# huangnengCSU/NanoSNP

Hardware: AMD Instinct MI355X
Metric: candidate SNP sites/sec (pileup encode + model fwd), 30x windows (higher is better)
Workload: dtype f32; 1 GPU; BASELINE configs[1]: pileup encode + PileupModel fwd, 1M synthetic 30x windows (G2) resident in HBM, batch=4096; batch=4096, windows_resident_per_gpu=1048576, streams=32, precision=fp32, parallelism=site-sharded x1, rooted gather of calls, world_size_observed=1, gather=torch

## Files before the change

nanosnp_amd/csrc/nsnp_api.hip:

```cpp
#include "nsnp_common.hpp"

#include <new>

extern "C" int nsnp_version(void) { return 101; }

extern "C" const char* nsnp_strerror(int code)
{
    switch (code) {
    case NSNP_OK: return "ok";
    case NSNP_EINVAL: return "invalid argument";
    case NSNP_ENOMEM: return "out of memory";
    case NSNP_EHIP: return "HIP runtime error";
    case NSNP_ENOWEIGHTS: return "weights not loaded";
    case NSNP_EARCH: return "device is not gfx950";
    case NSNP_ESHAPE: return "unsupported model dimensions";
    case NSNP_ENOTSUP: return "optional component unavailable (RCCL not found)";
    case NSNP_ECOMM: return "RCCL call failed";
    default: return "unknown error";
    }
}

static hipError_t g_create_err = hipSuccess;

extern "C" int nsnp_last_hip_error(const nsnp_ctx* ctx, const char** text)
{
    const hipError_t e = ctx ? ctx->last_err : g_create_err;
    if (text) *text = hipGetErrorString(e);
    return (int)e;
}

extern "C" int nsnp_ctx_create(int device, nsnp_ctx** out)
{
    if (!out) return NSNP_EINVAL;
    *out = nullptr;
    nsnp_ctx* ctx = new (std::nothrow) nsnp_ctx();
    if (!ctx) return NSNP_ENOMEM;
    memset((void*)ctx, 0, sizeof(*ctx));
    ctx->device = device;
    ctx->last_err = hipSuccess;
    ctx->chunk_sites = 32768;
    ctx->hap_chunk = 16384;
    ctx->precision = 0;
    ctx->hap_precision = 0;
    ctx->cat_precision = 0;
    ctx->cat_conv_lds = 1;
    ctx->cat_conv_pix2 = 1;
    ctx->hap_b3x = 1;
    ctx->tok_fused = 0;
    ctx->proj1_tiles = 4;
    ctx->fused_l1 = 1;
    ctx->l0_rs = 2;
    ctx->l0_weave = 1;
    ctx->l0_prestage = 1;
    ctx->l1_rs = 1;
    ctx->l1_stagger = 0;
    ctx->l1_weave = 1;
    ctx->head_rs = 1;
    ctx->rs_prio = 0;
    hipDeviceProp_t prop;
    hipError_t e = hipSetDevice(device);
    if (e == hipSuccess) e = hipGetDeviceProperties(&prop, device);
    if (e != hipSuccess) { g_create_err = e; delete ctx; return NSNP_EHIP; }
    if (strncmp(prop.gcnArchName, "gfx950", 6) != 0) { delete ctx; return NSNP_EARCH; }
    ctx->n_cu = prop.multiProcessorCount;
    *out = ctx;
    return NSNP_OK;
}

void nsnp_hap_free(nsnp_ctx* ctx);
int  nsnp_hap_reserve(nsnp_ctx* ctx);
void nsnp_cat_free(nsnp_ctx* ctx);
void nsnp_tok_free(nsnp_ctx* ctx);
void nsnp_train_free(nsnp_ctx* ctx);

constexpr size_t TIMER_MAX_PAIRS = 8192;

ScopedKernelTimer::ScopedKernelTimer(nsnp_ctx* c, int kernel, hipStream_t stream)
    : ctx(c), k(kernel), s(stream), stop_ev(nullptr), on(false)
{
    KernelTimer* t = c->timer;
    if (!t || !t->enabled || t->used[k] >= TIMER_MAX_PAIRS) return;
    if (t->used[k] == t->start[k].size()) {
        hipEvent_t a, b;
        if (hipEventCreate(&a) != hipSuccess) return;
        if (hipEventCreate(&b) != hipSuccess) { (void)hipEventDestroy(a); return; }
        t->start[k].push_back(a); t->stop[k].push_back(b);
    }
    const size_t i = t->used[k]++;
    (void)hipEventRecord(t->start[k][i], s);
    stop_ev = t->stop[k][i];
    on = true;
}
void ScopedKernelTimer::stop() { if (on) { (void)hipEventRecord(stop_ev, s); on = false; } }
ScopedKernelTimer::~ScopedKernelTimer() { stop(); }

extern "C" int nsnp_ctx_set_option(nsnp_ctx* ctx, const char* name, int64_t value)
{
    if (!ctx || !name) return NSNP_EINVAL;
    if (strcmp(name, "cat_precision") == 0) {
        if (value != 0 && value != 1 && value != 2) return NSNP_EINVAL;
        ctx->cat_precision = (int)value;
        return NSNP_OK;
    }
    if (strcmp(name, "tok_fused") == 0) {
        if (value != 0 && value != 1) return NSNP_EINVAL;
        ctx->tok_fused = (int)value;
        return NSNP_OK;
    }
    if (strcmp(name, "hap_b3x") == 0) {
        if (value != 0 && value != 1) return NSNP_EINVAL;
        ctx->hap_b3x = (int)value;
        return NSNP_OK;
    }
    if (strcmp(name, "cat_conv_pix2") == 0) {
        if (value != 0 && value != 1) return NSNP_EINVAL;
        ctx->cat_conv_pix2 = (int)value;
        return NSNP_OK;
    }
    if (strcmp(name, "cat_conv_lds") == 0) {
        if (value != 0 && value != 1) return NSNP_EINVAL;
        ctx->cat_conv_lds = (int)value;
        return NSNP_OK;
    }
    if (strcmp(name, "hap_precision") == 0) {
        if (value != 0 && value != 1 && value != 2) return NSNP_EINVAL;
        ctx->hap_precision = (int)value;
        return nsnp_hap_reserve(ctx);
    }
    if (strcmp(name, "hap_pass_sites") == 0) {
        if (value < 128 || value > 131072 || value % 128) return NSNP_EINVAL;
        const int64_t old = ctx->hap_chunk;
        ctx->hap_chunk = value;
        const int rc = nsnp_hap_reserve(ctx);
        if (rc) { ctx->hap_chunk = old; (void)nsnp_hap_reserve(ctx); }
        return rc;
    }
    if (strcmp(name, "pileup_precision") == 0) {
        if (value != 0 && value != 1 && value != 2) return NSNP_EINVAL;
        ctx->precision = (int)value;
        if (value == 2 && ctx->ws_h0 && ctx->ws_h0_floats < 192) return nsnp_ctx_reserve(ctx, ctx->chunk_sites);
        return NSNP_OK;
    }
    if (strcmp(name, "fused_l1") == 0) {
        if (value != 0 && value != 1) return NSNP_EINVAL;
        ctx->fused_l1 = (int)value;
        return NSNP_OK;
    }
    if (strcmp(name, "l0_register_stationary") == 0) {
        if (value != 0 && value != 1 && value != 2) return NSNP_EINVAL;
        ctx->l0_rs = (int)value;
        return NSNP_OK;
    }
    if (strcmp(name, "l1_register_stationary") == 0) {
        if (value != 0 && value != 1 && value != 2) return NSNP_EINVAL;
        ctx->l1_rs = (int)value;
        return NSNP_OK;
    }
    if (strcmp(name, "l0_input_weights_in_lds") == 0) {
        if (value != 0 && value != 1) return NSNP_EINVAL;
        ctx->l0_wx_lds = (int)value;
        return NSNP_OK;
    }
    if (strcmp(name, "static_priority") == 0) {
        if (value < 0 || value > 3) return NSNP_EINVAL;
        ctx->rs_prio = (int)value;
        return NSNP_OK;
    }
    if (strcmp(name, "head_split") == 0) {
        if (value != 0 && value != 1) return NSNP_EINVAL;
        ctx->head_rs = (int)value;
        return NSNP_OK;
    }
    if (strcmp(name, "l1_stagger") == 0) {
        if (value != 0 && value != 1) return NSNP_EINVAL;
        ctx->l1_stagger = (int)value;
        return NSNP_OK;
    }
    if (strcmp(name, "l1_weave") == 0) {
        if (value != 0 && value != 1) return NSNP_EINVAL;
        ctx->l1_weave = (int)value;
        return NSNP_OK;
    }
    if (strcmp(name, "l0_weave") == 0) {
        if (value != 0 && value != 1) return NSNP_EINVAL;
        ctx->l0_weave = (int)value;
        return NSNP_OK;
    }
    if (strcmp(name, "l0_prestage") == 0) {
        if (value != 0 && value != 1) return NSNP_EINVAL;
        ctx->l0_prestage = (int)value;
        return NSNP_OK;
    }
    if (strcmp(name, "l1_site_groups") == 0) {
        if (value != 0 && value != 1 && value != 2 && value != 4) return NSNP_EINVAL;
        ctx->l1_rs_groups = (int)value;
        return NSNP_OK;
    }
    if (strcmp(name, "l0_site_groups") == 0) {
        if (value != 0 && value != 1 && value != 2 && value != 4) return NSNP_EINVAL;
        ctx->l0_rs_groups = (int)value;
        return NSNP_OK;
    }
    if (strcmp(name, "fused_waves") == 0) {
        if (value != 0 && value != 4 && value != 8 && value != 12) return NSNP_EINVAL;
        ctx->fused_waves = (int)value;
        return NSNP_OK;
    }
    if (strcmp(name, "proj1_tiles") == 0) {
        if (value < 1 || value > 64) return NSNP_EINVAL;
        ctx->proj1_tiles = (int)value;
        return NSNP_OK;
    }
    if (strcmp(name, "recurrence_waves") == 0) {
        if (value != 0 && value != 1 && value != 2 && value != 4 && value != 8) return NSNP_EINVAL;
        ctx->force_wpb = (int)value;
        return NSNP_OK;
    }
    return NSNP_EINVAL;
}

extern "C" int nsnp_ctx_enable_timing(nsnp_ctx* ctx, int enable)
{
    if (!ctx) return NSNP_EINVAL;
    if (!ctx->timer) {
        ctx->timer = new (std::nothrow) KernelTimer();
        if (!ctx->timer) return NSNP_ENOMEM;
        for (int k = 0; k < NSNP_K_COUNT; ++k) ctx->timer->used[k] = 0;
    }
    ctx->timer->enabled = enable != 0;
    return NSNP_OK;
}

extern "C" int nsnp_ctx_read_timing(nsnp_ctx* ctx, int kernel, double* total_ms, int64_t* launches)
{
    if (!ctx || kernel < 0 || kernel >= NSNP_K_COUNT || !total_ms || !launches) return NSNP_EINVAL;
    *total_ms = 0.0; *launches = 0;
    KernelTimer* t = ctx->timer;
    if (!t) return NSNP_OK;
    for (size_t i = 0; i < t->used[kernel]; ++i) {
        NSNP_HIP(ctx, hipEventSynchronize(t->stop[kernel][i]));
        float ms = 0.f;
        NSNP_HIP(ctx, hipEventElapsedTime(&ms, t->start[kernel][i], t->stop[kernel][i]));
        *total_ms += ms; ++*launches;
    }
    t->used[kernel] = 0;
    return NSNP_OK;
}

static void free_ws(nsnp_ctx* ctx)
{
    if (ctx->ws_h0) (void)hipFree(ctx->ws_h0);
    if (ctx->ws_xp1) (void)hipFree(ctx->ws_xp1);
    if (ctx->ws_h1c) (void)hipFree(ctx->ws_h1c);
// ... 158 lines not shown
```

nanosnp_amd/csrc/nsnp_common.hpp:

```cpp
#pragma once

#include <hip/hip_runtime.h>
#include <stdint.h>
#include <stdlib.h>
#include <string.h>
#include <vector>

#include "nanosnp.h"

typedef float f32x4 __attribute__((ext_vector_type(4)));
typedef int   i32x4 __attribute__((ext_vector_type(4)));

#define NSNP_CDIV(a, b) (((a) + (b) - 1) / (b))

constexpr int PW = NSNP_PILEUP_WINDOW;
constexpr int PC = NSNP_PILEUP_CHANNELS;
constexpr int PH = 64;
constexpr int PG = 4 * PH;
constexpr int PCENTER = 16;
constexpr int PSTEPS1 = PCENTER + 1;


struct PileupWeightsDev {
    float* l0_whh[2];
    float* l0_wih[2];
    float* l0_wlast[2];
    void*  l0_wx[2];
    float* l1_wih[2];
    float* l1_bias[2];
    float* l1_bias_raw[2];
    float* l1_whh[2];
    float* proj_w;
    float* proj_b;
    float* dense_w;
    float* dense_b;
    float* head_w;
    float* head_b;
    float* arena;
    size_t arena_bytes;
    bool   loaded;
    float* head6_w;
    float* head6_b;
    bool   indel_loaded;
};

struct PileupWeightsF16 {
    void* l0_whh[2]; void* l0_wih_hi[2]; void* l0_wih_lo[2]; void* l1_wih[2]; void* l1_whh[2];
    void* l1f_hi[2]; void* l1f_lo[2]; float* l1f_bias;
    void* l0_wih_rs[2];
    void* l1_wih_rs[2]; void* l1_whh_rs[2];
    void* l0_whh_rs[2];
    void* proj_w; void* dense_w; void* head_w;
    void* arena; size_t arena_bytes; bool loaded;
};

struct PileupWeightsB3 {
    void* l0_whh[2]; void* l0_wih[2]; void* l1_wih[2]; void* l1_whh[2];
    void* proj_w; void* dense_w; void* head_w;
    float* proj_b; float* dense_b; float* head_b;
    void* arena; size_t arena_bytes; bool loaded;
};

struct HapWeightsDev;
struct CatWeightsDev;

enum { NSNP_K_L0 = 0, NSNP_K_PROJ1, NSNP_K_L1, NSNP_K_HEAD, NSNP_K_ENCODE, NSNP_K_HAPFEAT, NSNP_K_HAPLSTM, NSNP_K_CATCONV, NSNP_K_CAT,
       NSNP_K_HAPHEAD,
       NSNP_K_TRAIN_FWD, NSNP_K_TRAIN_BWD, NSNP_K_TRAIN_WGRAD,
       NSNP_K_COUNT };
struct KernelTimer {
    std::vector<hipEvent_t> start[NSNP_K_COUNT], stop[NSNP_K_COUNT];
    size_t used[NSNP_K_COUNT];
    bool enabled;
};

struct PostOut { uint8_t* gt_arg; uint8_t* zy_arg; float* gt_max; float* zy_max; };

struct nsnp_ctx {
    int device;
    int n_cu;
    hipError_t last_err;
    bool attr_set;
    bool attr_set_f16;
    bool attr_set_b3;
    int hap_b3x;
    int cat_conv_pix2;
    int cat_conv_lds;
    int cat_precision;
    int hap_precision;
    int precision;
    int fused_waves;
    int l0_rs;
    int l1_rs_groups;
    int l1_rs;
    int l0_rs_groups;
    int fused_l1;
    int proj1_tiles;
    int force_wpb;
    int l0_wx_lds;
    int rs_prio;
    int head_rs;
    int l1_stagger;
    int l0_weave;
    int l0_prestage;
    int l1_weave;
    int64_t chunk_sites;
    float*  ws_h0;
    int     ws_h0_floats;
    float*  ws_xp1;
    float*  ws_h1c;
    PileupWeightsDev pw;
    PileupWeightsF16 pw16;
    PileupWeightsB3 pwb3;
    HapWeightsDev* hw;
    void*  hap_ws; size_t hap_ws_bytes; int64_t hap_ws_chunk;
    int64_t hap_chunk;
    CatWeightsDev* cw;
    void*  cat_ws; size_t cat_ws_bytes;
    int64_t* sel_tmp; size_t sel_tmp_bytes;
    int64_t* fil_tmp; size_t fil_tmp_bytes;
    void* rec_tmp; size_t rec_tmp_bytes;
    void* evl_tmp; size_t evl_tmp_bytes;
    void* tr_ws; int64_t tr_sites;
    void* lab_tmp; size_t lab_tmp_bytes;
    void* tok_ws; size_t tok_ws_bytes;
    void* ctg_ws; size_t ctg_ws_bytes;
    int tok_fused;
    bool af_cached; uint64_t af_bits, af_t; int af_k, af_mode; uint32_t af_table_words[128];
    bool af2_cached; uint64_t af2_bits, af2_t; int af2_k, af2_mode; uint32_t af2_table_words[128];
    KernelTimer* timer;
    void* comm; int comm_rank, comm_world;
    bool comm_borrowed;
};

struct ScopedKernelTimer {
    nsnp_ctx* ctx; int k; hipStream_t s; hipEvent_t stop_ev; bool on;
    ScopedKernelTimer(nsnp_ctx* c, int kernel, hipStream_t stream);
    void stop();
    ~ScopedKernelTimer();
};

#define NSNP_HIP(ctx, call)                                                        \
    do {                                                                           \
        hipError_t e_ = (call);                                                    \
        if (e_ != hipSuccess) { (ctx)->last_err = e_; return NSNP_EHIP; }          \
    } while (0)

typedef float (*nsnp_wfun)(const void* user, int row, int k);
void nsnp_pack_image(float* img, int n_tiles, int n_j4, nsnp_wfun f, const void* user);

int nsnp_ctx_need_xp1(nsnp_ctx* ctx);

int nsnp_pileup_forward_impl(nsnp_ctx* ctx, const int32_t* x, const int64_t* center_idx,
                             int64_t N, float* gt, float* zy, const PostOut* post, bool* post_written, hipStream_t s);
int nsnp_pileup_pack_weights(nsnp_ctx* ctx, const float* const* w);
int nsnp_pileup_pack_indel_heads(nsnp_ctx* ctx, const float* const* w);
int nsnp_pileup_eval_impl(nsnp_ctx* ctx, const int32_t* x, const int64_t* center_idx, const uint8_t* cls, int64_t N, float* site_loss,
                          uint8_t* pred, int64_t* counters, float* logits, hipStream_t s);
void nsnp_pileup_eval_heads_launch(nsnp_ctx* ctx, int64_t n, const uint8_t* cls, float* site_loss, uint8_t* pred, int64_t* counters,
                                   float* logits, hipStream_t s);
int nsnp_hap_dims(const nsnp_ctx* ctx, int* n_gt, int* n_zy);
int nsnp_pileup_forward_f16x3(nsnp_ctx* ctx, const int32_t* x, const int64_t* center_idx,
                              int64_t N, float* gt, float* zy, hipStream_t s);
int nsnp_pileup_pack_weights_f16(nsnp_ctx* ctx, const float* const* w);
int nsnp_pileup_forward_bf16x3(nsnp_ctx* ctx, const int32_t* x, const int64_t* center_idx, int64_t N, float* gt, float* zy,
                               const PostOut* post, hipStream_t s);
int nsnp_pileup_pack_weights_bf16(nsnp_ctx* ctx, const float* const* w);
```

nanosnp_amd/csrc/pileup_forward.hip:

```cpp
#include "nsnp_common.hpp"
#include "nsnp_lstm_cell.hpp"
#include "nsnp_devclock.hpp"
#include "nsnp_bf16.hpp"
#include <type_traits>

namespace {

constexpr float LOG2E = 1.4426950408889634f;

__device__ __forceinline__ f32x4 mfma4(float a, float b, f32x4 c)
{
    return __builtin_amdgcn_mfma_f32_16x16x4f32(a, b, c, 0, 0, 0);
}
__device__ __forceinline__ float sigmoid_f(float x)
{
    return __builtin_amdgcn_rcpf(1.0f + __builtin_amdgcn_exp2f(-LOG2E * x));
}
__device__ __forceinline__ float tanh_f(float x)
{
    return __builtin_fmaf(-2.0f, __builtin_amdgcn_rcpf(1.0f + __builtin_amdgcn_exp2f((2.0f * LOG2E) * x)), 1.0f);
}

__device__ __forceinline__ float lstm_cell(float zi, float zf, float zg, float zo, float& c)
{
// ... 1526 lines not shown
        for (int u = 0; u < 2; ++u)
#pragma unroll
            for (int g = 0; g < 4; ++g) x2[4 * (2 * wave + u) + g][lane] = tanh_f(ad[u][g]);
        __syncthreads();
        f32x4 ah = bh;
        if (wave < 2) {
#pragma unroll
            for (int j = 0; j < 16; ++j)
#pragma unroll
                for (int e = 0; e < 4; ++e) ah = mfma4(Wh[j][e], x2[4 * j + e][lane], ah);
            if (wave == 1) x3[lane] = ah;
        }
        __syncthreads();
        if (wave == 0) {
            const f32x4 a1 = x3[lane];
            const float NEG = -3.0e38f;
            float g0[4], g1[4];
#pragma unroll
            for (int g = 0; g < 4; ++g) {
                g0[g] = ah[g];
                const bool is_gt = (q == 0) || (q == 1 && g == 0);
                g1[g] = is_gt ? a1[g] : NEG;
            }
            float mx = fmaxf(fmaxf(fmaxf(g0[0], g0[1]), fmaxf(g0[2], g0[3])), fmaxf(fmaxf(g1[0], g1[1]), fmaxf(g1[2], g1[3])));
            mx = fmaxf(mx, __shfl_xor(mx, 16));
            mx = fmaxf(mx, __shfl_xor(mx, 32));
            float e0[4], e1[4], sum = 0.f;
#pragma unroll
            for (int g = 0; g < 4; ++g) {
                e0[g] = __expf(g0[g] - mx);
                e1[g] = g1[g] > -1.0e38f ? __expf(g1[g] - mx) : 0.f;
                sum += e0[g] + e1[g];
            }
            sum += __shfl_xor(sum, 16);
            sum += __shfl_xor(sum, 32);
            const float z1 = a1[1], z2 = a1[2], z3 = a1[3];
            const float zm = fmaxf(z1, fmaxf(z2, z3));
            const float ez1 = __expf(z1 - zm), ez2 = __expf(z2 - zm), ez3 = __expf(z3 - zm);
            const float zs = ez1 + ez2 + ez3;
            float p0[4], p1[4];
#pragma unroll
            for (int g = 0; g < 4; ++g) { p0[g] = e0[g] / sum; p1[g] = e1[g] / sum; }
            const float pz1 = ez1 / zs, pz2 = ez2 / zs, pz3 = ez3 / zs;
            if (live) {
                float* gp = gt_prob + site * NSNP_GT_CLASSES;
#pragma unroll
                for (int g = 0; g < 4; ++g) gp[4 * q + g] = p0[g];
                if (q == 0) {
#pragma unroll
                    for (int g = 0; g < 4; ++g) gp[16 + g] = p1[g];
                }
                if (q == 1) {
                    gp[20] = p1[0];
                    float* zp = zy_prob + site * NSNP_ZY_CLASSES;
                    zp[0] = pz1; zp[1] = pz2; zp[2] = pz3;
                }
            }
            if (gt_arg) {
                float bv = p0[0]; int bi = 4 * q;
#pragma unroll
                for (int g = 1; g < 4; ++g) if (p0[g] > bv) { bv = p0[g]; bi = 4 * q + g; }
                if (q == 0) {
#pragma unroll
                    for (int g = 0; g < 4; ++g) if (p1[g] > bv) { bv = p1[g]; bi = 16 + g; }
                }
                if (q == 1 && p1[0] > bv) { bv = p1[0]; bi = 20; }
#pragma unroll
                for (int o = 16; o <= 32; o <<= 1) {
                    const float ov = __shfl_xor(bv, o); const int oi = __shfl_xor(bi, o);
                    if (ov > bv || (ov == bv && oi < bi)) { bv = ov; bi = oi; }
                }
                if (live && q == 0) { gt_arg[site] = (uint8_t)bi; gt_max[site] = bv; }
                if (live && q == 1) {
                    float zb = pz1; int zi = 0;
                    if (pz2 > zb) { zb = pz2; zi = 1; }
                    if (pz3 > zb) { zb = pz3; zi = 2; }
                    zy_arg[site] = (uint8_t)zi; zy_max[site] = zb;
                }
            }
        }
    }
}

__global__ void k_pileup_post(const float* __restrict__ gt, const float* __restrict__ zy,
                              const int32_t* __restrict__ x, int64_t N, uint8_t* gt_arg, uint8_t* zy_arg,
                              float* gt_max, float* zy_max, int32_t* depth)
{
    const int64_t n = (int64_t)blockIdx.x * blockDim.x + threadIdx.x;
    if (n >= N) return;
    const float* g = gt + n * NSNP_GT_CLASSES;
    int bi = 0; float bv = g[0];
    for (int i = 1; i < NSNP_GT_CLASSES; ++i) if (g[i] > bv) { bv = g[i]; bi = i; }
    gt_arg[n] = (uint8_t)bi; gt_max[n] = bv;
    const float* z = zy + n * NSNP_ZY_CLASSES;
    bi = 0; bv = z[0];
    for (int i = 1; i < NSNP_ZY_CLASSES; ++i) if (z[i] > bv) { bv = z[i]; bi = i; }
    zy_arg[n] = (uint8_t)bi; zy_max[n] = bv;
    if (depth) {
        const int32_t* c = x + n * (PW * PC) + PCENTER * PC;
        const int idx[8] = {0, 1, 2, 3, 9, 10, 11, 12};
        int d = 0;
        for (int k = 0; k < 8; ++k) { const int v = c[idx[k]]; if (v < 0) d -= v; }
        depth[n] = d;
    }
}

}

namespace {

inline int gate_row(int row)
{
    const int i = row >> 4, r = row & 15, qp = r >> 2, g = r & 3;
    return g * PH + 4 * i + qp;
}
struct MatRef { const float* w; int ld; const float* b0; const float* b1; };

float f_whh(const void* u, int row, int k) { const MatRef* m = (const MatRef*)u; return m->w[gate_row(row) * m->ld + k]; }
float f_wih0(const void* u, int row, int k) { const MatRef* m = (const MatRef*)u; return m->w[gate_row(row) * m->ld + k]; }
inline int h_store_col(int k) { const int j = k >> 2, q = k & 3; return (j >> 4) * 64 + 4 * (j & 15) + q; }
float f_wih1(const void* u, int row, int k) { const MatRef* m = (const MatRef*)u; return m->w[gate_row(row) * m->ld + h_store_col(k)]; }
float f_proj(const void* u, int row, int k) { const MatRef* m = (const MatRef*)u; return m->w[row * m->ld + h_store_col(k)]; }
inline int acc_col(int k) { const int j = k >> 2, q = k & 3; return 16 * (j >> 2) + 4 * q + (j & 3); }
float f_dense(const void* u, int row, int k) { const MatRef* m = (const MatRef*)u; return m->w[row * m->ld + acc_col(k)]; }
struct HeadRef { const float* gt; const float* zy; };
float f_head(const void* u, int row, int k)
{
    const HeadRef* m = (const HeadRef*)u;
    if (row < 21) return m->gt[row * 256 + acc_col(k)];
    if (row < 24) return m->zy[(row - 21) * 256 + acc_col(k)];
    return 0.f;
}

}

void nsnp_pack_image(float* img, int n_tiles, int n_j4, nsnp_wfun f, const void* user)
{
    for (int tile = 0; tile < n_tiles; ++tile)
        for (int j4 = 0; j4 < n_j4; ++j4)
            for (int lane = 0; lane < 64; ++lane)
                for (int e = 0; e < 4; ++e) {
                    const int row = 16 * tile + (lane & 15);
                    const int k = 4 * (4 * j4 + e) + (lane >> 4);
                    img[(((size_t)tile * n_j4 + j4) * 64 + lane) * 4 + e] = f(user, row, k);
                }
}

int nsnp_pileup_pack_weights(nsnp_ctx* ctx, const float* const* w)
{
    PileupWeightsDev& pw = ctx->pw;
    const size_t n_whh = 16 * 4 * 256, n_wih0 = 16 * 1 * 256, n_wlast = 16 * 64, n_wih1 = 16 * 8 * 256,
                 n_b1 = 16 * 256, n_proj = 8 * 8 * 256, n_pb = 8 * 256, n_dense = 16 * 8 * 256, n_db = 16 * 256,
                 n_head = 2 * 16 * 256, n_hb = 2 * 256;
    const size_t n_wx = 16 * 3 * 64 * 8 / 2;
    const size_t total = 2 * (n_whh + n_wih0 + n_wlast + n_wx + n_wih1 + 2 * n_b1 + n_whh) + n_proj + n_pb + n_dense + n_db + n_head + n_hb;
    std::vector<float> host(total);
    size_t off = 0;
    auto take = [&](size_t n) { float* p = host.data() + off; off += n; return p; };
    float* h_l0_whh[2]; float* h_l0_wih[2]; float* h_l0_wlast[2]; float* h_l0_wx[2];
    float* h_l1_wih[2]; float* h_l1_b[2]; float* h_l1_braw[2]; float* h_l1_whh[2];
    for (int d = 0; d < 2; ++d) {
        h_l0_whh[d] = take(n_whh); h_l0_wih[d] = take(n_wih0); h_l0_wlast[d] = take(n_wlast); h_l0_wx[d] = take(n_wx);
        h_l1_wih[d] = take(n_wih1); h_l1_b[d] = take(n_b1); h_l1_braw[d] = take(n_b1); h_l1_whh[d] = take(n_whh);
    }
    float* h_proj = take(n_proj); float* h_pb = take(n_pb); float* h_dense = take(n_dense); float* h_db = take(n_db);
    float* h_head = take(n_head); float* h_hb = take(n_hb);
// ... 20 lines not shown
            for (int lane = 0; lane < 64; ++lane) {
                const int tr = gate_row(16 * tile + (lane & 15)), kq = lane >> 4;
                float v = 0.f;
                if (kq < 2) v = l0[0][tr * PC + 16 + kq];
                else if (kq == 2) v = l0[2][tr] + l0[3][tr];
                h_l0_wlast[d][tile * 64 + lane] = v;
            }
        pack_b3(reinterpret_cast<uint16_t*>(h_l0_wx[d]), 16, 1, [&](int row, int, int q, int j) {
            const int k = 8 * q + j, tr = gate_row(row);
            return k < PC ? l0[0][tr * PC + k] : (k == PC ? l0[2][tr] + l0[3][tr] : 0.f);
        });
        m = MatRef{l1[0], 2 * PH, nullptr, nullptr};  nsnp_pack_image(h_l1_wih[d], 16, 8, f_wih1, &m);
        for (int tile = 0; tile < 16; ++tile)
            for (int lane = 0; lane < 64; ++lane)
                for (int g = 0; g < 4; ++g) {
                    const int tr = gate_row(16 * tile + 4 * (lane >> 4) + g);
                    h_l1_b[d][(tile * 64 + lane) * 4 + g] = l1[2][tr] + l1[3][tr];
                    h_l1_braw[d][(tile * 64 + lane) * 4 + g] = w[8 + d * 4 + 2][tr] + w[8 + d * 4 + 3][tr];
                }
        m = MatRef{l1[1], PH, nullptr, nullptr};  nsnp_pack_image(h_l1_whh[d], 16, 4, f_whh, &m);
    }
    {
        MatRef m{w[16], 128, nullptr, nullptr};  nsnp_pack_image(h_proj, 8, 8, f_proj, &m);
        for (int tile = 0; tile < 8; ++tile) for (int lane = 0; lane < 64; ++lane) for (int g = 0; g < 4; ++g)
            h_pb[(tile * 64 + lane) * 4 + g] = w[17][16 * tile + 4 * (lane >> 4) + g];
        MatRef md{w[18], 128, nullptr, nullptr}; nsnp_pack_image(h_dense, 16, 8, f_dense, &md);
        for (int tile = 0; tile < 16; ++tile) for (int lane = 0; lane < 64; ++lane) for (int g = 0; g < 4; ++g)
            h_db[(tile * 64 + lane) * 4 + g] = w[19][16 * tile + 4 * (lane >> 4) + g];
        HeadRef hr{w[20], w[22]};  nsnp_pack_image(h_head, 2, 16, f_head, &hr);
        for (int tile = 0; tile < 2; ++tile) for (int lane = 0; lane < 64; ++lane) for (int g = 0; g < 4; ++g) {
            const int row = 16 * tile + 4 * (lane >> 4) + g;
            h_hb[(tile * 64 + lane) * 4 + g] = row < 21 ? w[21][row] : (row < 24 ? w[23][row - 21] : 0.f);
        }
    }
    if (pw.arena && pw.arena_bytes != total * sizeof(float)) { (void)hipFree(pw.arena); pw.arena = nullptr; }
    if (!pw.arena) {
        NSNP_HIP(ctx, hipMalloc((void**)&pw.arena, total * sizeof(float)));
        pw.arena_bytes = total * sizeof(float);
    }
    NSNP_HIP(ctx, hipMemcpy(pw.arena, host.data(), total * sizeof(float), hipMemcpyHostToDevice));
    auto dev = [&](const float* hp) { return pw.arena + (hp - host.data()); };
    for (int d = 0; d < 2; ++d) {
        pw.l0_whh[d] = dev(h_l0_whh[d]); pw.l0_wih[d] = dev(h_l0_wih[d]); pw.l0_wlast[d] = dev(h_l0_wlast[d]);
        pw.l0_wx[d] = dev(h_l0_wx[d]);
        pw.l1_wih[d] = dev(h_l1_wih[d]); pw.l1_bias[d] = dev(h_l1_b[d]); pw.l1_bias_raw[d] = dev(h_l1_braw[d]); pw.l1_whh[d] = dev(h_l1_whh[d]);
    }
    pw.proj_w = dev(h_proj); pw.proj_b = dev(h_pb); pw.dense_w = dev(h_dense); pw.dense_b = dev(h_db);
    pw.head_w = dev(h_head); pw.head_b = dev(h_hb);
    pw.loaded = true;
    pw.indel_loaded = false;
    return NSNP_OK;
}

int nsnp_pileup_pack_indel_heads(nsnp_ctx* ctx, const float* const* w)
{
    PileupWeightsDev& pw = ctx->pw;
    constexpr size_t n_w = 6 * 16 * 256, n_b = 6 * 256;
    std::vector<float> img(n_w), bias(n_b), old_w(2 * 16 * 256), old_b(2 * 256);
    NSNP_HIP(ctx, hipDeviceSynchronize());
    NSNP_HIP(ctx, hipMemcpy(old_w.data(), pw.head_w, old_w.size() * sizeof(float), hipMemcpyDeviceToHost));
    NSNP_HIP(ctx, hipMemcpy(old_b.data(), pw.head_b, old_b.size() * sizeof(float), hipMemcpyDeviceToHost));
    struct IndelRef { const float* w1; const float* w2; } ir{w[0], w[2]};
    nsnp_pack_image(img.data(), 6, 16, [](const void* u, int row, int k) -> float {
        const IndelRef* m = (const IndelRef*)u;
        if (row >= 24 && row < 57) return m->w1[(row - 24) * 256 + acc_col(k)];
        if (row >= 57 && row < 90) return m->w2[(row - 57) * 256 + acc_col(k)];
        return 0.f;
    }, &ir);
    for (int tile = 0; tile < 2; ++tile) for (int j4 = 0; j4 < 16; ++j4) for (int lane = 0; lane < 64; ++lane)
        if (16 * tile + (lane & 15) < 24)
            for (int e = 0; e < 4; ++e) img[((tile * 16 + j4) * 64 + lane) * 4 + e] = old_w[((tile * 16 + j4) * 64 + lane) * 4 + e];
    for (int tile = 0; tile < 6; ++tile) for (int lane = 0; lane < 64; ++lane) for (int g = 0; g < 4; ++g) {
        const int row = 16 * tile + 4 * (lane >> 4) + g;
        bias[(tile * 64 + lane) * 4 + g] = row < 24 ? old_b[(tile * 64 + lane) * 4 + g] : (row < 57 ? w[1][row - 24] : (row < 90 ? w[3][row - 57] : 0.f));
    }
    if (!pw.head6_w) NSNP_HIP(ctx, hipMalloc((void**)&pw.head6_w, n_w * sizeof(float)));
    if (!pw.head6_b) NSNP_HIP(ctx, hipMalloc((void**)&pw.head6_b, n_b * sizeof(float)));
    NSNP_HIP(ctx, hipMemcpy(pw.head6_w, img.data(), n_w * sizeof(float), hipMemcpyHostToDevice));
    NSNP_HIP(ctx, hipMemcpy(pw.head6_b, bias.data(), n_b * sizeof(float), hipMemcpyHostToDevice));
    pw.indel_loaded = true;
    return NSNP_OK;
}

static int set_lds_attr_once(nsnp_ctx* ctx)
{
    if (ctx->attr_set) return NSNP_OK;
    NSNP_HIP(ctx, hipFuncSetAttribute((const void*)k_pileup_l0<8>, hipFuncAttributeMaxDynamicSharedMemorySize, L0_LDS_BYTES));
    NSNP_HIP(ctx, hipFuncSetAttribute((const void*)k_pileup_l0<4>, hipFuncAttributeMaxDynamicSharedMemorySize, L0_LDS_BYTES));
    NSNP_HIP(ctx, hipFuncSetAttribute((const void*)k_pileup_l0<2>, hipFuncAttributeMaxDynamicSharedMemorySize, L0_LDS_BYTES));
    NSNP_HIP(ctx, hipFuncSetAttribute((const void*)k_pileup_l0<1>, hipFuncAttributeMaxDynamicSharedMemorySize, L0_LDS_BYTES));
    NSNP_HIP(ctx, hipFuncSetAttribute((const void*)k_pileup_proj1, hipFuncAttributeMaxDynamicSharedMemorySize, P1_LDS_BYTES));
    NSNP_HIP(ctx, hipFuncSetAttribute((const void*)k_pileup_l1<8>, hipFuncAttributeMaxDynamicSharedMemorySize, L1_LDS_BYTES));
    NSNP_HIP(ctx, hipFuncSetAttribute((const void*)k_pileup_l1<4>, hipFuncAttributeMaxDynamicSharedMemorySize, L1_LDS_BYTES));
    NSNP_HIP(ctx, hipFuncSetAttribute((const void*)k_pileup_l1<2>, hipFuncAttributeMaxDynamicSharedMemorySize, L1_LDS_BYTES));
    NSNP_HIP(ctx, hipFuncSetAttribute((const void*)k_pileup_l1<1>, hipFuncAttributeMaxDynamicSharedMemorySize, L1_LDS_BYTES));
    NSNP_HIP(ctx, hipFuncSetAttribute((const void*)k_pileup_l1_rs4<1>, hipFuncAttributeMaxDynamicSharedMemorySize, rs4_l1_lds_bytes(1)));
    NSNP_HIP(ctx, hipFuncSetAttribute((const void*)k_pileup_l1_rs4<2>, hipFuncAttributeMaxDynamicSharedMemorySize, rs4_l1_lds_bytes(2)));
    NSNP_HIP(ctx, hipFuncSetAttribute((const void*)k_pileup_l1_rs4w<RS4W_PER_GAP, RS4W_FIRST_GAP>, hipFuncAttributeMaxDynamicSharedMemorySize, rs4w_l1_lds_bytes()));
    NSNP_HIP(ctx, hipFuncSetAttribute((const void*)k_pileup_l1_rs32<4, true>, hipFuncAttributeMaxDynamicSharedMemorySize, rs32_l1_lds_bytes(4)));
    NSNP_HIP(ctx, hipFuncSetAttribute((const void*)k_pileup_l1_rs32<2, true>, hipFuncAttributeMaxDynamicSharedMemorySize, rs32_l1_lds_bytes(2)));
    NSNP_HIP(ctx, hipFuncSetAttribute((const void*)k_pileup_l1_rs32<4, false>, hipFuncAttributeMaxDynamicSharedMemorySize, rs32_l1_lds_bytes(4)));
    NSNP_HIP(ctx, hipFuncSetAttribute((const void*)k_pileup_l1_rs32<2, false>, hipFuncAttributeMaxDynamicSharedMemorySize, rs32_l1_lds_bytes(2)));
    ctx->attr_set = true;
    return NSNP_OK;
}

static int launch_layers(nsnp_ctx* ctx, const int32_t* xc, const int64_t* cc, int64_t n, hipStream_t s)
{
    const PileupWeightsDev& pw = ctx->pw;
    {
        const int64_t waves_total = NSNP_CDIV(n, 16) * 2;
        int wpb = 8;
        while (wpb > 1 && waves_total / wpb < (int64_t)ctx->n_cu / 2) wpb >>= 1;
        if (ctx->force_wpb) wpb = ctx->force_wpb;
        const dim3 g_rec((unsigned)NSNP_CDIV(n, 16 * wpb), 2);
        if (ctx->l0_rs == 2) {
            ScopedKernelTimer tm(ctx, NSNP_K_L0, s);
            if (ctx->l0_weave && ctx->l0_prestage)
                hipLaunchKernelGGL((k_pileup_l0_rsxp<RSXW_GAP_T, RSXW_GAP_V, RSXW_GAP_FIRST, RSXW_LATE_W0 != 0>), dim3((unsigned)NSNP_CDIV(n, 16), 2), dim3(256), 0, s,
                                   xc, cc, n, pw.l0_whh[0], pw.l0_whh[1], (const __bf16*)pw.l0_wx[0], (const __bf16*)pw.l0_wx[1], ctx->ws_h0);
            else if (ctx->l0_weave)
                hipLaunchKernelGGL((k_pileup_l0_rsxw<RSXW_GAP_T, RSXW_GAP_V, RSXW_GAP_FIRST, RSXW_LATE_W0 != 0>), dim3((unsigned)NSNP_CDIV(n, 16), 2), dim3(256), 0, s,
                                   xc, cc, n, pw.l0_whh[0], pw.l0_whh[1], (const __bf16*)pw.l0_wx[0], (const __bf16*)pw.l0_wx[1], ctx->ws_h0);
            else
            hipLaunchKernelGGL(k_pileup_l0_rsx, dim3((unsigned)NSNP_CDIV(n, 16), 2), dim3(256), 0, s, xc, cc, n,
                               pw.l0_whh[0], pw.l0_whh[1], (const __bf16*)pw.l0_wx[0], (const __bf16*)pw.l0_wx[1], ctx->ws_h0);
        } else if (ctx->l0_rs) {
            ScopedKernelTimer tm(ctx, NSNP_K_L0, s);
            int nsg = 1;
            if (ctx->l0_rs_groups) nsg = ctx->l0_rs_groups;
#define LAUNCH_RS(G) hipLaunchKernelGGL(k_pileup_l0_rs32<G>, dim3((unsigned)NSNP_CDIV(n, 16 * G), 2), dim3(256), 0, s, xc, cc, n, \
                           pw.l0_whh[0], pw.l0_whh[1], pw.l0_wih[0], pw.l0_wih[1], pw.l0_wlast[0], pw.l0_wlast[1], ctx->ws_h0)
            if (ctx->l0_wx_lds && nsg == 1)
                hipLaunchKernelGGL((k_pileup_l0_rs32<1, true>), dim3((unsigned)NSNP_CDIV(n, 16), 2), dim3(256), 0, s, xc, cc, n,
                                   pw.l0_whh[0], pw.l0_whh[1], pw.l0_wih[0], pw.l0_wih[1], pw.l0_wlast[0], pw.l0_wlast[1], ctx->ws_h0);
            else
            if (nsg == 4) LAUNCH_RS(4); else if (nsg == 2) LAUNCH_RS(2); else LAUNCH_RS(1);
#undef LAUNCH_RS
        } else
        { ScopedKernelTimer tm(ctx, NSNP_K_L0, s);
#define LAUNCH_L0(W) hipLaunchKernelGGL(k_pileup_l0<W>, g_rec, dim3(64 * W), L0_LDS_BYTES, s, xc, cc, n, \
                           pw.l0_whh[0], pw.l0_whh[1], pw.l0_wih[0], pw.l0_wih[1], pw.l0_wlast[0], pw.l0_wlast[1], ctx->ws_h0)
        if (wpb == 8) LAUNCH_L0(8); else if (wpb == 4) LAUNCH_L0(4); else if (wpb == 2) LAUNCH_L0(2); else LAUNCH_L0(1);
#undef LAUNCH_L0
        }
        if (ctx->l1_rs == 1) {
            ScopedKernelTimer tm(ctx, NSNP_K_L1, s);
            int g1 = 1;
            if (ctx->l1_rs_groups == 1 || ctx->l1_rs_groups == 2) g1 = ctx->l1_rs_groups;
#define LAUNCH_R4(G) hipLaunchKernelGGL(k_pileup_l1_rs4<G>, dim3((unsigned)NSNP_CDIV(n, 16 * G), 2), dim3(256), rs4_l1_lds_bytes(G), s, \
                           ctx->ws_h0, n, pw.l1_wih[0], pw.l1_wih[1], pw.l1_whh[0], pw.l1_whh[1], pw.l1_bias[0], pw.l1_bias[1], ctx->ws_h1c)
            if (g1 == 2) LAUNCH_R4(2);
            else if (ctx->l1_weave)
                hipLaunchKernelGGL((k_pileup_l1_rs4w<RS4W_PER_GAP, RS4W_FIRST_GAP>), dim3((unsigned)NSNP_CDIV(n, 16), 2), dim3(256),
                                   rs4w_l1_lds_bytes(), s, ctx->ws_h0, n, pw.l1_wih[0], pw.l1_wih[1], pw.l1_whh[0], pw.l1_whh[1],
                                   pw.l1_bias[0], pw.l1_bias[1], ctx->ws_h1c);
            else LAUNCH_R4(1);
#undef LAUNCH_R4
        } else if (ctx->l1_rs == 2) {
            ScopedKernelTimer tm(ctx, NSNP_K_L1, s);
            int g1 = NSNP_CDIV(n, 64) * 2 >= (int64_t)ctx->n_cu ? 4 : 2;
            if (ctx->l1_rs_groups) g1 = ctx->l1_rs_groups;
#define LAUNCH_R1(G) hipLaunchKernelGGL((k_pileup_l1_rs32<G, ST>), dim3((unsigned)NSNP_CDIV(n, 16 * G), 2), dim3(512), rs32_l1_lds_bytes(G), s, \
                           ctx->ws_h0, n, pw.l1_wih[0], pw.l1_wih[1], pw.l1_whh[0], pw.l1_whh[1], pw.l1_bias[0], pw.l1_bias[1], ctx->ws_h1c)
            if (ctx->l1_stagger) { constexpr bool ST = true; if (g1 == 4) LAUNCH_R1(4); else LAUNCH_R1(2); }
            else { constexpr bool ST = false; if (g1 == 4) LAUNCH_R1(4); else LAUNCH_R1(2); }
#undef LAUNCH_R1
        } else {
        { const int rx = nsnp_ctx_need_xp1(ctx); if (rx) return rx; }
        const int64_t n_rt = NSNP_CDIV(n * PSTEPS1, 16);
        int64_t gp = NSNP_CDIV(n_rt, 16 * (int64_t)ctx->proj1_tiles);
        if (gp > ctx->n_cu) gp = ctx->n_cu;
        if (gp < 1) gp = 1;
        { ScopedKernelTimer tm(ctx, NSNP_K_PROJ1, s);
        hipLaunchKernelGGL(k_pileup_proj1, dim3((unsigned)gp, 2), dim3(1024), P1_LDS_BYTES, s, ctx->ws_h0, n,
                           pw.l1_wih[0], pw.l1_wih[1], pw.l1_bias[0], pw.l1_bias[1], ctx->ws_xp1); }
        { ScopedKernelTimer tm(ctx, NSNP_K_L1, s);
#define LAUNCH_L1(W) hipLaunchKernelGGL(k_pileup_l1<W>, g_rec, dim3(64 * W), L1_LDS_BYTES, s, ctx->ws_xp1, n, \
                           pw.l1_whh[0], pw.l1_whh[1], ctx->ws_h1c)
        if (wpb == 8) LAUNCH_L1(8); else if (wpb == 4) LAUNCH_L1(4); else if (wpb == 2) LAUNCH_L1(2); else LAUNCH_L1(1);
#undef LAUNCH_L1
        }
        }
    }
    return NSNP_OK;
}

int nsnp_pileup_forward_impl(nsnp_ctx* ctx, const int32_t* x, const int64_t* center_idx,
                             int64_t N, float* gt, float* zy, const PostOut* post, bool* post_written, hipStream_t s)
{
    if (!ctx->pw.loaded) return NSNP_ENOWEIGHTS;
    if (N == 0) return NSNP_OK;
    int rc = set_lds_attr_once(ctx);
    if (rc) return rc;
    if (!ctx->ws_h0) { rc = nsnp_ctx_reserve(ctx, ctx->chunk_sites); if (rc) return rc; }
    const PileupWeightsDev& pw = ctx->pw;
    for (int64_t base = 0; base < N; base += ctx->chunk_sites) {
        const int64_t n = (N - base < ctx->chunk_sites) ? N - base : ctx->chunk_sites;
        const int32_t* xc = center_idx ? x : x + base * (PW * PC);
        const int64_t* cc = center_idx ? center_idx + base : nullptr;
        rc = launch_layers(ctx, xc, cc, n, s);
        if (rc) return rc;
        ScopedKernelTimer tm_head(ctx, NSNP_K_HEAD, s);
        if (ctx->head_rs) {
            int64_t gh = NSNP_CDIV(n, 16);
            if (gh > 2 * (int64_t)ctx->n_cu) gh = 2 * (int64_t)ctx->n_cu;
            const PostOut po = post ? *post : PostOut{nullptr, nullptr, nullptr, nullptr};
            hipLaunchKernelGGL(k_pileup_head_rs, dim3((unsigned)gh), dim3(512), 0, s, ctx->ws_h1c, n,
                               pw.proj_w, pw.proj_b, pw.dense_w, pw.dense_b, pw.head_w, pw.head_b,
                               gt + base * NSNP_GT_CLASSES, zy + base * NSNP_ZY_CLASSES,
                               po.gt_arg ? po.gt_arg + base : nullptr, po.gt_arg ? po.zy_arg + base : nullptr,
                               po.gt_arg ? po.gt_max + base : nullptr, po.gt_arg ? po.zy_max + base : nullptr);
            if (post_written) *post_written = po.gt_arg != nullptr;
        } else
        hipLaunchKernelGGL(k_pileup_head, dim3((unsigned)NSNP_CDIV(n, 64)), dim3(256), 0, s, ctx->ws_h1c, n,
                           pw.proj_w, pw.proj_b, pw.dense_w, pw.dense_b, pw.head_w, pw.head_b,
                           gt + base * NSNP_GT_CLASSES, zy + base * NSNP_ZY_CLASSES);
    }
    NSNP_HIP(ctx, hipGetLastError());
    return NSNP_OK;
}

int nsnp_pileup_eval_impl(nsnp_ctx* ctx, const int32_t* x, const int64_t* center_idx, const uint8_t* cls, int64_t N, float* site_loss,
                          uint8_t* pred, int64_t* counters, float* logits, hipStream_t s)
{
    if (!ctx->pw.loaded || !ctx->pw.indel_loaded) return NSNP_ENOWEIGHTS;
    if (N == 0) return NSNP_OK;
    int rc = set_lds_attr_once(ctx);
    if (rc) return rc;
    if (!ctx->ws_h0) { rc = nsnp_ctx_reserve(ctx, ctx->chunk_sites); if (rc) return rc; }
    for (int64_t base = 0; base < N; base += ctx->chunk_sites) {
        const int64_t n = (N - base < ctx->chunk_sites) ? N - base : ctx->chunk_sites;
        rc = launch_layers(ctx, center_idx ? x : x + base * (PW * PC), center_idx ? center_idx + base : nullptr, n, s);
        if (rc) return rc;
        ScopedKernelTimer tm_head(ctx, NSNP_K_HEAD, s);
        nsnp_pileup_eval_heads_launch(ctx, n, cls ? cls + base * 4 : nullptr, cls ? site_loss + base * 4 : nullptr, cls ? pred + base * 4 : nullptr,
                                      counters, logits ? logits + base * NSNP_LABEL_WIDTH : nullptr, s);
    }
    NSNP_HIP(ctx, hipGetLastError());
    return NSNP_OK;
}

NSNP_DEVCLK_READER(nsnp_devclk_read_pileup)

extern "C" int nsnp_pileup_postprocess(nsnp_ctx* ctx, const float* gt_prob, const float* zy_prob,
                                       const int32_t* x, int64_t N, uint8_t* gt_arg, uint8_t* zy_arg,
                                       float* gt_max, float* zy_max, int32_t* depth, void* stream)
{
    if (!ctx || N < 0 || (N > 0 && (!gt_prob || !zy_prob || !gt_arg || !zy_arg || !gt_max || !zy_max || (depth && !x)))) return NSNP_EINVAL;
    if (N == 0) return NSNP_OK;
    hipLaunchKernelGGL(k_pileup_post, dim3((unsigned)NSNP_CDIV(N, 256)), dim3(256), 0, (hipStream_t)stream,
                       gt_prob, zy_prob, x, N, gt_arg, zy_arg, gt_max, zy_max, depth);
    NSNP_HIP(ctx, hipGetLastError());
    return NSNP_OK;
}
```

Baseline: 21.51 million sites/s.

## Process multiple 16-site groups per head block to amortize stationary weights

Adds a templated head kernel that processes NG site groups (2 or 4) per iteration, interleaving MFMAs across groups while reusing the register-resident proj/dense/head weights. Head-output work is spread across 2*NG waves and softmax/argmax finishing is factored into a helper. By default, chunks larger than 16 sites use two groups per block, and a tunable knob selects 1, 2 or 4. The aim is more independent MFMA chains and better latency hiding in the head, at the cost of extra LDS, more registers and fewer blocks in the grid.

```diff
diff --git a/nanosnp_amd/csrc/nsnp_api.hip b/nanosnp_amd/csrc/nsnp_api.hip
--- a/nanosnp_amd/csrc/nsnp_api.hip
+++ b/nanosnp_amd/csrc/nsnp_api.hip
@@ -56,6 +56,7 @@
     ctx->l1_stagger = 0;
     ctx->l1_weave = 1;
     ctx->head_rs = 1;
+    ctx->head_groups = 0;
     ctx->rs_prio = 0;
     hipDeviceProp_t prop;
     hipError_t e = hipSetDevice(device);
@@ -169,6 +170,11 @@
     if (strcmp(name, "head_split") == 0) {
         if (value != 0 && value != 1) return NSNP_EINVAL;
         ctx->head_rs = (int)value;
+        return NSNP_OK;
+    }
+    if (strcmp(name, "head_groups") == 0) {
+        if (value != 0 && value != 1 && value != 2 && value != 4) return NSNP_EINVAL;
+        ctx->head_groups = (int)value;
         return NSNP_OK;
     }
     if (strcmp(name, "l1_stagger") == 0) {
diff --git a/nanosnp_amd/csrc/nsnp_common.hpp b/nanosnp_amd/csrc/nsnp_common.hpp
--- a/nanosnp_amd/csrc/nsnp_common.hpp
+++ b/nanosnp_amd/csrc/nsnp_common.hpp
@@ -100,6 +100,7 @@
     int l0_wx_lds;
     int rs_prio;
     int head_rs;
+    int head_groups;
     int l1_stagger;
     int l0_weave;
     int l0_prestage;
diff --git a/nanosnp_amd/csrc/pileup_forward.hip b/nanosnp_amd/csrc/pileup_forward.hip
--- a/nanosnp_amd/csrc/pileup_forward.hip
+++ b/nanosnp_amd/csrc/pileup_forward.hip
@@ -1632,6 +1632,199 @@
     }
 }
 
+__device__ __forceinline__ void head_finish(const f32x4 a0, const f32x4 a1, const int q, const bool live, const int64_t site,
+                                            float* __restrict__ gt_prob, float* __restrict__ zy_prob, uint8_t* __restrict__ gt_arg,
+                                            uint8_t* __restrict__ zy_arg, float* __restrict__ gt_max, float* __restrict__ zy_max)
+{
+    const float NEG = -3.0e38f;
+    float g0[4], g1[4];
+#pragma unroll
+    for (int g = 0; g < 4; ++g) {
+        g0[g] = a0[g];
+        const bool is_gt = (q == 0) || (q == 1 && g == 0);
+        g1[g] = is_gt ? a1[g] : NEG;
+    }
+    float mx = fmaxf(fmaxf(fmaxf(g0[0], g0[1]), fmaxf(g0[2], g0[3])), fmaxf(fmaxf(g1[0], g1[1]), fmaxf(g1[2], g1[3])));
+    mx = fmaxf(mx, __shfl_xor(mx, 16));
+    mx = fmaxf(mx, __shfl_xor(mx, 32));
+    float e0[4], e1[4], sum = 0.f;
+#pragma unroll
+    for (int g = 0; g < 4; ++g) {
+        e0[g] = __expf(g0[g] - mx);
+        e1[g] = g1[g] > -1.0e38f ? __expf(g1[g] - mx) : 0.f;
+        sum += e0[g] + e1[g];
+    }
+    sum += __shfl_xor(sum, 16);
+    sum += __shfl_xor(sum, 32);
+    const float z1 = a1[1], z2 = a1[2], z3 = a1[3];
+    const float zm = fmaxf(z1, fmaxf(z2, z3));
+    const float ez1 = __expf(z1 - zm), ez2 = __expf(z2 - zm), ez3 = __expf(z3 - zm);
+    const float zs = ez1 + ez2 + ez3;
+    float p0[4], p1[4];
+#pragma unroll
+    for (int g = 0; g < 4; ++g) { p0[g] = e0[g] / sum; p1[g] = e1[g] / sum; }
+    const float pz1 = ez1 / zs, pz2 = ez2 / zs, pz3 = ez3 / zs;
+    if (live) {
+        float* gp = gt_prob + site * NSNP_GT_CLASSES;
+#pragma unroll
+        for (int g = 0; g < 4; ++g) gp[4 * q + g] = p0[g];
+        if (q == 0) {
+#pragma unroll
+            for (int g = 0; g < 4; ++g) gp[16 + g] = p1[g];
+        }
+        if (q == 1) {
+            gp[20] = p1[0];
+            float* zp = zy_prob + site * NSNP_ZY_CLASSES;
+            zp[0] = pz1; zp[1] = pz2; zp[2] = pz3;
+        }
+    }
+    if (gt_arg) {
+        float bv = p0[0]; int bi = 4 * q;
+#pragma unroll
+        for (int g = 1; g < 4; ++g) if (p0[g] > bv) { bv = p0[g]; bi = 4 * q + g; }
+        if (q == 0) {
+#pragma unroll
+            for (int g = 0; g < 4; ++g) if (p1[g] > bv) { bv = p1[g]; bi = 16 + g; }
+        }
+        if (q == 1 && p1[0] > bv) { bv = p1[0]; bi = 20; }
+#pragma unroll
+        for (int o = 16; o <= 32; o <<= 1) {
+            const float ov = __shfl_xor(bv, o); const int oi = __shfl_xor(bi, o);
+            if (ov > bv || (ov == bv && oi < bi)) { bv = ov; bi = oi; }
+        }
+        if (live && q == 0) { gt_arg[site] = (uint8_t)bi; gt_max[site] = bv; }
+        if (live && q == 1) {
+            float zb = pz1; int zi = 0;
+            if (pz2 > zb) { zb = pz2; zi = 1; }
+            if (pz3 > zb) { zb = pz3; zi = 2; }
+            zy_arg[site] = (uint8_t)zi; zy_max[site] = zb;
+        }
+    }
+}
+
+constexpr int head_rsg_lds_bytes(int ng) { return ng * (32 * 64 + 64 * 64) * 4 + ng * 2 * 64 * 16 + 8 * 4 * 64 * 16; }
+
+template <int NG>
+__global__ __launch_bounds__(512) void k_pileup_head_rsg(
+    const float* __restrict__ H1c, int64_t N,
+    const float* __restrict__ proj_w, const float* __restrict__ proj_b,
+    const float* __restrict__ dense_w, const float* __restrict__ dense_b,
+    const float* __restrict__ head_w, const float* __restrict__ head_b,
+    float* __restrict__ gt_prob, float* __restrict__ zy_prob,
+    uint8_t* __restrict__ gt_arg, uint8_t* __restrict__ zy_arg, float* __restrict__ gt_max, float* __restrict__ zy_max)
+{
+    static_assert(NG == 2 || NG == 4, "head tiles are spread over waves 0 .. 2 NG - 1 of eight");
+    extern __shared__ f32x4 lds[];
+    float* const x1 = reinterpret_cast<float*>(lds);
+    float* const x2 = x1 + NG * 32 * 64;
+    f32x4* const x3 = reinterpret_cast<f32x4*>(x2 + NG * 64 * 64);
+    const int tid = threadIdx.x, lane = tid & 63, wave = tid >> 6;
+    f32x4* const xb = x3 + NG * 2 * 64 + wave * 4 * 64 + lane;
+    const int q = lane >> 4;
+    const bool has_head = wave < 2 * NG;
+    const int ht = wave & 1, hg = wave >> 1;
+    const f32x4* const pw = reinterpret_cast<const f32x4*>(proj_w);
+    const f32x4* const dw = reinterpret_cast<const f32x4*>(dense_w);
+    const f32x4* const hw = reinterpret_cast<const f32x4*>(head_w);
+    f32x4 Wp[8], Wd[2][8], Wh[16];
+    const int64_t n_groups = NSNP_CDIV(N, 16), n_sets = NSNP_CDIV(n_groups, NG);
+
+    auto do_set = [&](const int64_t set, auto first_tag) {
+        constexpr bool FIRST = decltype(first_tag)::value;
+        const f32x4* __restrict__ hin[NG];
+#pragma unroll
+        for (int g = 0; g < NG; ++g) {
+            const int64_t site = (set * NG + g) * 16 + (lane & 15);
+            const int64_t sc = site < N ? site : N - 1;
+            hin[g] = reinterpret_cast<const f32x4*>(H1c + sc * 128 + q * 16);
+        }
+        constexpr int HJ = NG == 2 ? 4 : 2;
+        f32x4 hb[NG][HJ];
+#pragma unroll
+        for (int g = 0; g < NG; ++g)
+#pragma unroll
+            for (int j = 0; j < HJ; ++j) hb[g][j] = hin[g][j];
+        if constexpr (FIRST) {
+#pragma unroll
+            for (int j = 0; j < 8; ++j) Wp[j] = pw[(wave * 8 + j) * 64 + lane];
+            xb[0] = reinterpret_cast<const f32x4*>(proj_b)[wave * 64 + lane];
+#pragma unroll
+            for (int j = 0; j < 8; ++j) {
+                Wd[0][j] = dw[((2 * wave) * 8 + j) * 64 + lane];
+                Wd[1][j] = dw[((2 * wave + 1) * 8 + j) * 64 + lane];
+            }
+            xb[64] = reinterpret_cast<const f32x4*>(dense_b)[(2 * wave) * 64 + lane];
+            xb[128] = reinterpret_cast<const f32x4*>(dense_b)[(2 * wave + 1) * 64 + lane];
+        }
+        f32x4 ap[NG];
+#pragma unroll
+        for (int g = 0; g < NG; ++g) ap[g] = xb[0];
+#pragma unroll
+        for (int h = 0; h < 8 / HJ; ++h) {
+            if (h > 0) {
+#pragma unroll
+                for (int g = 0; g < NG; ++g)
+#pragma unroll
+                    for (int j = 0; j < HJ; ++j) { const int jj = h * HJ + j; hb[g][j] = hin[g][(jj >> 2) * 16 + (jj & 3)]; }
+            }
+#pragma unroll
+            for (int j = 0; j < HJ; ++j)
+#pragma unroll
+                for (int e = 0; e < 4; ++e)
+#pragma unroll
+                    for (int g = 0; g < NG; ++g) ap[g] = mfma4(Wp[h * HJ + j][e], hb[g][j][e], ap[g]);
+        }
+        if constexpr (FIRST) {
+            if (has_head) {
+#pragma unroll
+                for (int j = 0; j < 16; ++j) Wh[j] = hw[(ht * 16 + j) * 64 + lane];
+                xb[192] = reinterpret_cast<const f32x4*>(head_b)[ht * 64 + lane];
+            }
+        }
+#pragma unroll
+        for (int g = 0; g < NG; ++g)
+#pragma unroll
+            for (int r = 0; r < 4; ++r) x1[(g * 32 + 4 * wave + r) * 64 + lane] = ap[g][r];
+        __syncthreads();
+        f32x4 ad[NG][2];
+#pragma unroll
+        for (int g = 0; g < NG; ++g) { ad[g][0] = xb[64]; ad[g][1] = xb[128]; }
+#pragma unroll
+        for (int j = 0; j < 8; ++j)
+#pragma unroll
+            for (int e = 0; e < 4; ++e)
+#pragma unroll
+                for (int g = 0; g < NG; ++g) {
+                    const float b = x1[(g * 32 + 4 * j + e) * 64 + lane];
+                    ad[g][0] = mfma4(Wd[0][j][e], b, ad[g][0]);
+                    ad[g][1] = mfma4(Wd[1][j][e], b, ad[g][1]);
+                }
+#pragma unroll
+        for (int g = 0; g < NG; ++g)
+#pragma unroll
+            for (int u = 0; u < 2; ++u)
+#pragma unroll
+                for (int r = 0; r < 4; ++r) x2[(g * 64 + 4 * (2 * wave + u) + r) * 64 + lane] = tanh_f(ad[g][u][r]);
+        __syncthreads();
+        if (has_head) {
+            f32x4 ah = xb[192];
+#pragma unroll
+            for (int j = 0; j < 16; ++j)
+#pragma unroll
+                for (int e = 0; e < 4; ++e) ah = mfma4(Wh[j][e], x2[(hg * 64 + 4 * j + e) * 64 + lane], ah);
+            x3[(hg * 2 + ht) * 64 + lane] = ah;
+        }
+        __syncthreads();
+        if (wave < NG) {
+            const int64_t site = (set * NG + wave) * 16 + (lane & 15);
+            head_finish(x3[(wave * 2) * 64 + lane], x3[(wave * 2 + 1) * 64 + lane], q, site < N, site,
+                        gt_prob, zy_prob, gt_arg, zy_arg, gt_max, zy_max);
+        }
+    };
+    do_set((int64_t)blockIdx.x, std::true_type{});
+    for (int64_t set = (int64_t)blockIdx.x + gridDim.x; set < n_sets; set += gridDim.x) do_set(set, std::false_type{});
+}
+
 __global__ void k_pileup_post(const float* __restrict__ gt, const float* __restrict__ zy,
                               const int32_t* __restrict__ x, int64_t N, uint8_t* gt_arg, uint8_t* zy_arg,
                               float* gt_max, float* zy_max, int32_t* depth)
@@ -1818,6 +2011,11 @@
     return NSNP_OK;
 }
 
+static int head_groups_rule(int64_t n)
+{
+    return n > 16 ? 2 : 1;
+}
+
 static int set_lds_attr_once(nsnp_ctx* ctx)
 {
     if (ctx->attr_set) return NSNP_OK;
@@ -1837,6 +2035,8 @@
     NSNP_HIP(ctx, hipFuncSetAttribute((const void*)k_pileup_l1_rs32<2, true>, hipFuncAttributeMaxDynamicSharedMemorySize, rs32_l1_lds_bytes(2)));
     NSNP_HIP(ctx, hipFuncSetAttribute((const void*)k_pileup_l1_rs32<4, false>, hipFuncAttributeMaxDynamicSharedMemorySize, rs32_l1_lds_bytes(4)));
     NSNP_HIP(ctx, hipFuncSetAttribute((const void*)k_pileup_l1_rs32<2, false>, hipFuncAttributeMaxDynamicSharedMemorySize, rs32_l1_lds_bytes(2)));
+    NSNP_HIP(ctx, hipFuncSetAttribute((const void*)k_pileup_head_rsg<2>, hipFuncAttributeMaxDynamicSharedMemorySize, head_rsg_lds_bytes(2)));
+    NSNP_HIP(ctx, hipFuncSetAttribute((const void*)k_pileup_head_rsg<4>, hipFuncAttributeMaxDynamicSharedMemorySize, head_rsg_lds_bytes(4)));
     ctx->attr_set = true;
     return NSNP_OK;
 }
@@ -1939,14 +2139,19 @@
         if (rc) return rc;
         ScopedKernelTimer tm_head(ctx, NSNP_K_HEAD, s);
         if (ctx->head_rs) {
-            int64_t gh = NSNP_CDIV(n, 16);
+            const int ng = ctx->head_groups ? ctx->head_groups : head_groups_rule(n);
+            int64_t gh = NSNP_CDIV(NSNP_CDIV(n, 16), ng);
             if (gh > 2 * (int64_t)ctx->n_cu) gh = 2 * (int64_t)ctx->n_cu;
             const PostOut po = post ? *post : PostOut{nullptr, nullptr, nullptr, nullptr};
-            hipLaunchKernelGGL(k_pileup_head_rs, dim3((unsigned)gh), dim3(512), 0, s, ctx->ws_h1c, n,
-                               pw.proj_w, pw.proj_b, pw.dense_w, pw.dense_b, pw.head_w, pw.head_b,
-                               gt + base * NSNP_GT_CLASSES, zy + base * NSNP_ZY_CLASSES,
-                               po.gt_arg ? po.gt_arg + base : nullptr, po.gt_arg ? po.zy_arg + base : nullptr,
-                               po.gt_arg ? po.gt_max + base : nullptr, po.gt_arg ? po.zy_max + base : nullptr);
+#define LAUNCH_HEAD(K, LDS) hipLaunchKernelGGL(K, dim3((unsigned)gh), dim3(512), LDS, s, ctx->ws_h1c, n, \
+                               pw.proj_w, pw.proj_b, pw.dense_w, pw.dense_b, pw.head_w, pw.head_b, \
+                               gt + base * NSNP_GT_CLASSES, zy + base * NSNP_ZY_CLASSES, \
+                               po.gt_arg ? po.gt_arg + base : nullptr, po.gt_arg ? po.zy_arg + base : nullptr, \
+                               po.gt_arg ? po.gt_max + base : nullptr, po.gt_arg ? po.zy_max + base : nullptr)
+            if (ng == 4) LAUNCH_HEAD(k_pileup_head_rsg<4>, head_rsg_lds_bytes(4));
+            else if (ng == 2) LAUNCH_HEAD(k_pileup_head_rsg<2>, head_rsg_lds_bytes(2));
+            else LAUNCH_HEAD(k_pileup_head_rs, 0);
+#undef LAUNCH_HEAD
             if (post_written) *post_written = po.gt_arg != nullptr;
         } else
         hipLaunchKernelGGL(k_pileup_head, dim3((unsigned)NSNP_CDIV(n, 64)), dim3(256), 0, s, ctx->ws_h1c, n,
```

Result: no change. 21.69 million sites/s, median of 6 (+0.8%).
